# micknoise/Maximilian

Measured on AMD Instinct MI355X. Metric: Msamples/s (voice-bank render), higher is better.
Workload: dtype f64; 1 GPU; configs[1]: 65536-voice maxiOsc::sinebuf bank, block 512, out[n][v] stored, 8 rotated buffers; voices_per_gpu=65536, block=512, parallelism=units sharded x1, mixdown=off

## Files before the change

### maximilian_amd/csrc/mxg_pace.h

```cpp
#pragma once
#include "mxg_common.h"

namespace mxg {
namespace {

constexpr int kPaceWords = 8;
constexpr unsigned kPaceWindow = 32, kPaceLatesUp = 4, kPaceLatesDown = 1;
constexpr unsigned kPaceGaveUp = 0xffffffffu;

struct Pace {
    unsigned P, t0, k, late, cheap;
    __device__ __forceinline__ static unsigned now() { return (unsigned)__builtin_amdgcn_s_memrealtime(); }
    __device__ __forceinline__ void start(const unsigned *ctl, unsigned arg) {
        P = arg;
        if (ctl) {
            const unsigned p = __hip_atomic_load(ctl, __ATOMIC_RELAXED, __HIP_MEMORY_SCOPE_AGENT);
            if (p == kPaceGaveUp) P = 0;
            else if (p) P = p < 2 * arg ? p : 2 * arg;
        }
        k = late = cheap = 0;
        t0 = P ? now() : 0;
    }
    __device__ __forceinline__ void wait(bool is_cheap) {
        if (P) {
            const unsigned due = t0 + k * P;
            int d = (int)(now() - due);
            while (d < 0) {
                __builtin_amdgcn_s_sleep(1);
                d = (int)(now() - due);
            }
            late = (unsigned)d;
            k++;
            cheap += is_cheap ? 1u : 0u;
        }
    }
    __device__ __forceinline__ void finish(unsigned *ctl, unsigned arg, unsigned wg, unsigned nwg, bool tolerant = false) const {
        if (!ctl || !P || (wg & 15u)) return;
        const unsigned nrep = (nwg + 15u) / 16u;
        unsigned long long *acc = reinterpret_cast<unsigned long long *>(ctl + 4);
        const unsigned long long mine = ((unsigned long long)(late < 8 * P ? late : 8 * P) << 32) | ((unsigned long long)(k && cheap * 8 >= k * 7 ? 1u : 0u) << 16) | 1ull;
        const unsigned long long all = atomicAdd(acc, mine) + mine;
        if ((unsigned)(all & 0xffffu) != nrep) return;
        atomicExch(acc, 0ull);
        const unsigned worst = (unsigned)(all >> 32) / nrep, bound = (unsigned)((all >> 16) & 0xffffu);
        const unsigned c1 = atomicAdd(&ctl[1], 0u);
        unsigned p = P, w = c1 & 0xff, lates = (c1 >> 8) & 0xff, booted = (c1 >> 16) & 0xff, strikes = c1 >> 24;
        const unsigned up = tolerant ? 2 * kPaceLatesUp : kPaceLatesUp, down = tolerant ? 4 * kPaceLatesDown : kPaceLatesDown;
        if (bound * 8 >= nrep * 7) {
            const bool is_late = worst > p / 2;
            if (booted != 1) {
                strikes = is_late ? strikes + 1 : 0;
                if (booted == 0) {
                    if (is_late) {
                        booted = 2;
                        strikes = 0;
                    } else if (p > arg - arg / 4 + 1) {
                        p -= 2;
                    }
                } else if (strikes >= (tolerant ? 2u : 1u)) {
                    p++;
                    booted = 1;
                } else if (!is_late && p > arg - arg / 4) {
                    p--;
                }
            } else {
                lates += is_late ? 1 : 0;
                ++w;
                if (lates >= up) {
                    p++;
                    w = lates = 0;
                } else if (w >= kPaceWindow) {
                    if (lates <= down && p > arg - arg / 4) p--;
                    w = lates = 0;
                }
            }
        }
        if (p > arg + arg / 2) p = kPaceGaveUp;
        atomicExch(&ctl[0], p);
        atomicExch(&ctl[1], w | (lates << 8) | (booted << 16) | (strikes << 24));
        atomicExch(&ctl[7], worst);
    }
};

constexpr unsigned kTrialPhase = 32, kTrialCandidates = 3, kTrialAgain = 16384 + 5 * kTrialPhase;

struct PaceTrial {
    unsigned t_begin, n, period, tag;
    unsigned verdict;
    __device__ __forceinline__ static unsigned candidate(unsigned arg, unsigned i) { return arg * (31u - 2u * i) / 32u; }
    __device__ __forceinline__ void start(const unsigned *T, unsigned arg, unsigned block_len) {
        t_begin = Pace::now();
        n = 0;
        period = 0;
        verdict = 0;
        tag = block_len & 0xffffu;
        if (T) {
            unsigned d = __hip_atomic_load(T, __ATOMIC_RELAXED, __HIP_MEMORY_SCOPE_AGENT);
            const unsigned w1 = __hip_atomic_load(T + 1, __ATOMIC_RELAXED, __HIP_MEMORY_SCOPE_AGENT);
            n = w1 & 0xffffu;
            if ((w1 >> 16) != tag) {
                n = 0;
                d = 0;
            }
            verdict = d;
            if (d) {
                period = d >= 2 ? (d < 2 * arg ? d : 2 * arg) : 0;
            } else {
                const unsigned ph = n / kTrialPhase;
                period = (ph >= 2 && ph < 2 + kTrialCandidates) ? candidate(arg, ph - 2) : 0;
            }
        }
    }
    __device__ __forceinline__ void finish(unsigned *T, unsigned arg, unsigned wg, unsigned nwg) const {
        if (!T || (wg & 15u)) return;
        if (verdict && n + 1 < kTrialAgain) {
            if (wg == 0) __hip_atomic_fetch_add(&T[1], 1u, __ATOMIC_RELAXED, __HIP_MEMORY_SCOPE_AGENT);
            return;
        }
        const unsigned nrep = (nwg + 15u) / 16u;
        unsigned long long *acc = reinterpret_cast<unsigned long long *>(T + 2);
        const unsigned long long all = atomicAdd(acc, 1ull) + 1ull;
        if ((unsigned)(all & 0xffffu) != nrep) return;
        atomicExch(acc, 0ull);
        unsigned d = atomicAdd(&T[0], 0u), nn = n + 1;
        if ((atomicAdd(&T[1], 0u) >> 16) != tag) d = 0;
        if (!d) {
            if (nn % kTrialPhase == 0) {
                const unsigned t_now = Pace::now(), ph = n / kTrialPhase, wall = t_now - atomicAdd(&T[8], 0u);
                atomicExch(&T[8], t_now);
                if (ph == 1) {
                    atomicExch(&T[4], wall);
                    atomicExch(&T[5], 0xffffffffu);
                    atomicExch(&T[6], 0u);
                } else if (ph >= 2) {
                    unsigned best = atomicAdd(&T[5], 0u), best_p = atomicAdd(&T[6], 0u);
                    const bool done = ph + 1 == 2 + kTrialCandidates;
                    if (wall < best) {
                        best = wall;
                        best_p = candidate(arg, ph - 2);
                        atomicExch(&T[5], best);
                        atomicExch(&T[6], best_p);
                    }
                    if (done) d = ((unsigned long long)best * 100 < (unsigned long long)atomicAdd(&T[4], 0u) * 98) ? best_p : 1u;
                }
            }
        } else if (nn >= kTrialAgain) {
            d = 0;
            nn = 0;
        }
        atomicExch(&T[0], d);
        atomicExch(&T[1], nn | (tag << 16));
    }
};

}
}
```

### maximilian_amd/csrc/osc.hip

```cpp
#include <type_traits>

#include "mxg_common.h"
#include "maxi_tables.h"
#include "mxg_sincos.h"
#include "mxg_osc.h"
#include "mxg_lanefold.h"
#include "mxg_pace.h"

namespace mxg {

namespace {

__device__ const double MAXI_SINE_TAB_D[MAXI_SINE_TAB_LEN] = MAXI_SINE_TAB_INIT;
__device__ const double MAXI_TRANS_TAB_D[MAXI_TRANS_TAB_LEN] = MAXI_TRANS_TAB_INIT;

__device__ const double MXG_SINTAB_D[MXG_SINTAB_LEN] = {MXG_SINTAB_VALUES};

template <int WF>
constexpr bool uses_sine() {
    return WF == MXG_OSC_SINEBUF || WF == MXG_OSC_SINEBUF4;
}
static_assert((kSineOddOff & 1) == 1 && kSineOddOff >= MAXI_SINE_TAB_LEN, "parity copy of the sine table");
static_assert(tab_copy<MXG_OSC_SINEBUF, 1>() >= MAXI_SINE_TAB_LEN, "sinebuf's table copy");
static_assert(tab_copy<MXG_OSC_SAWN, 1>() >= MAXI_TRANS_TAB_LEN, "sawn's table copy");
static_assert(kSb4Copy >= MAXI_SINE_TAB_LEN && (kSb4Copy - 2) * 8 > 255 * 8, "sinebuf4's table copies: disjoint, and out of a ds_read2_b64's reach");
template <int WF, int FL = 0>
constexpr int tab_len() {
    return (WF == MXG_OSC_SINEBUF4 && MXG_SB4_PAIRS) ? kSineOddOff + MAXI_SINE_TAB_LEN + 1
           : WF == MXG_OSC_SINEBUF4                  ? 4 * kSb4Copy
           : uses_sine<WF>()                         ? tab_copy<WF, FL>() + MAXI_SINE_TAB_LEN
                           : (WF == MXG_OSC_SAWN ? tab_copy<WF, FL>() + MAXI_TRANS_TAB_LEN
                                                 : ((WF == MXG_OSC_SINEWAVE || WF == MXG_OSC_COSWAVE) ? MXG_SINTAB_WIDE_LEN : 1));
}
template <int WF, int FL = 0>
__device__ __forceinline__ void load_tab(double *s_tab) {
    if constexpr (uses_sine<WF>()) {
        for (int i = threadIdx.x; i < MAXI_SINE_TAB_LEN; i += blockDim.x) {
            s_tab[i] = MAXI_SINE_TAB_D[i];
            if constexpr (WF == MXG_OSC_SINEBUF4 && MXG_SB4_PAIRS) s_tab[kSineOddOff + i] = MAXI_SINE_TAB_D[i];
            if constexpr (tab_copy<WF, FL>() != 0) s_tab[tab_copy<WF, FL>() + i] = MAXI_SINE_TAB_D[i];
            if constexpr (WF == MXG_OSC_SINEBUF4 && !MXG_SB4_PAIRS) {
                s_tab[kSb4Copy + i] = MAXI_SINE_TAB_D[i];
                s_tab[2 * kSb4Copy + i] = MAXI_SINE_TAB_D[i];
                s_tab[3 * kSb4Copy + i] = MAXI_SINE_TAB_D[i];
            }
        }
    } else if constexpr (WF == MXG_OSC_SAWN) {
        for (int i = threadIdx.x; i < MAXI_TRANS_TAB_LEN; i += blockDim.x) {
            s_tab[i] = MAXI_TRANS_TAB_D[i];
            if constexpr (tab_copy<WF, FL>() != 0) s_tab[tab_copy<WF, FL>() + i] = MAXI_TRANS_TAB_D[i];
        }
    } else if constexpr (WF == MXG_OSC_SINEWAVE || WF == MXG_OSC_COSWAVE) {
        for (int i = threadIdx.x; i < MXG_SINTAB_WIDE_LEN; i += blockDim.x) s_tab[i] = MXG_SINTAB_D[i & (MXG_SINTAB_LEN - 1)];
    }
}

template <int WF, int FL, int ST>
__device__ __forceinline__ void paced_chunk(Pace &pc, double &ph, double &hd, const OscPre &q, const double *s_tab, double *&o, size_t P) {
    double r[8];
    osc_tick_chunk<WF, 8, FL>(ph, hd, q, s_tab, s_tab, r);
#pragma unroll
    for (int u = 0; u < 8; u++) asm volatile("" : "+v"(r[u]));
    pc.wait(true);
#pragma unroll
    for (int u = 0; u < 8; u++) {
        store1<ST>(o, r[u]);
        o += P;
    }
    __builtin_amdgcn_sched_barrier(0);
}

template <int WF, bool FPS, int VPL, int ST, bool PX>
__global__ void osc_kernel(size_t V, size_t N, const double *__restrict__ freq,
                           const double *__restrict__ p1, const double *__restrict__ p2,
                           double *__restrict__ phase_io, double *__restrict__ hold_io,
                           double *__restrict__ out, double sr, PartSync psync, int xcd, int p1ps, int passes, size_t v_begin,
                           size_t v_end, size_t P, unsigned *__restrict__ pace_ctl, unsigned pace_arg, unsigned *__restrict__ trial) {
#ifndef MXG_K1_LEAN_MASK
#define MXG_K1_LEAN_MASK ((1 << MXG_OSC_SINEWAVE) | (1 << MXG_OSC_COSWAVE) | (1 << MXG_OSC_SINEBUF4) | (1 << MXG_OSC_SAWN))
#endif
    constexpr bool kLean = ((MXG_K1_LEAN_MASK >> WF) & 1) != 0;
    constexpr int kFL = kLean ? kTickLean : 0;
    __shared__ __attribute__((aligned(16))) double s_tab[tab_len<WF, kFL>()];
    constexpr bool kPre = tab_len<WF, kFL>() > 1;
    double ph0[VPL] = {}, hd0[VPL] = {}, f0[VPL] = {};
    if constexpr (kPre) {
        const size_t w0 = v_begin + ((size_t)xcd_block(blockIdx.x, gridDim.x, xcd) * blockDim.x + threadIdx.x) * VPL;
        const size_t wc = (w0 + VPL <= v_end) ? w0 : (v_end >= v_begin + VPL ? v_end - VPL : v_begin);
#pragma unroll
        for (int j = 0; j < VPL; j++) {
            const size_t w = wc + j < v_end ? wc + j : v_end - 1;
            ph0[j] = phase_io[w];
            hd0[j] = hold_io[w];
            f0[j] = FPS ? 0.0 : freq[w];
        }
    }
    if constexpr (tab_len<WF, kFL>() > 1) {
        load_tab<WF, kFL>(s_tab);
        __syncthreads();
    }
    for (int pass = 0; pass < passes; pass++) {
    const size_t v0 = v_begin + (((size_t)pass * gridDim.x + xcd_block(blockIdx.x, gridDim.x, xcd)) * blockDim.x + threadIdx.x) * VPL;
    if (v0 >= v_end) return;

    double ph[VPL], hd[VPL];
    OscPre q[VPL];
#pragma unroll
    for (int j = 0; j < VPL; j++) {
        const bool pre = kPre && pass == 0 && v0 + VPL <= v_end;
        ph[j] = pre ? ph0[j] : phase_io[v0 + j];
        hd[j] = pre ? hd0[j] : hold_io[v0 + j];
        double a = p1 ? p1[v0 + j] : 0.0, b = p2 ? p2[v0 + j] : 0.0;
        if constexpr (!FPS) {
            q[j] = osc_pre<WF>(pre ? f0[j] : freq[v0 + j], sr, a, b);
        } else {
            q[j].p1 = a;
            q[j].p2 = b;
        }
    }
    int *const part_ctr = gridDim.y > 1 ? part_counter(psync) : nullptr;
    if (blockIdx.y + 1 != gridDim.y) part_signal(part_ctr);
    const size_t plen = (N + gridDim.y - 1) / gridDim.y;
    const size_t nA = blockIdx.y * plen < N ? blockIdx.y * plen : N;
    const size_t nB = nA + plen < N ? nA + plen : N;
    if constexpr (!FPS) {
#pragma unroll 4
        for (size_t n = 0; n < nA; n++) {
#pragma unroll
            for (int j = 0; j < VPL; j++) osc_skip<WF>(ph[j], hd[j], q[j], s_tab, s_tab);
        }
    }
    double *o = out + nA * P + v0;
    const double *fp = freq + v0;
    const double *pp = (FPS && p1ps) ? p1 + v0 : nullptr;
#ifndef MXG_OSC_UNROLL
#define MXG_OSC_UNROLL 4
#endif

    bool trust = false;
    if constexpr ((WF == MXG_OSC_SINEWAVE || WF == MXG_OSC_COSWAVE) && !FPS) {
        bool ok = true;
#pragma unroll
        for (int j = 0; j < VPL; j++)
            ok = ok && q[j].inc >= 0.0 && q[j].inc < 1.0 && ph[j] >= 0.0 && ph[j] < 2.0 && (__double2hiint(ph[j]) | __double2hiint(q[j].inc)) >= 0;
        trust = __all(ok);
        if (trust) {
#pragma unroll
            for (int j = 0; j < VPL; j++) q[j].sk = sintab_k();
        }
    }
    PaceTrial tr;
    tr.start(trial, pace_arg, (unsigned)N);
    Pace pc;
    pc.start(trial ? nullptr : pace_ctl, trial ? tr.period : pace_arg);
    auto run = [&](auto trust_tag) {
        constexpr bool kTrust = decltype(trust_tag)::value;
        size_t n = nA;
        if constexpr (PX && VPL == 1 && !FPS) {
            double *op = out + (nA + (threadIdx.x & 1)) * P + (v0 & ~(size_t)1);
            if constexpr (!kLean) {
                if (pc.P) {
                    double *o8 = out + nA * P + v0;
                    for (; n + 8 <= nB; n += 8) paced_chunk<WF, kFL, 1>(pc, ph[0], hd[0], q[0], s_tab, o8, P);
                    op += (n - nA) * P;
                }
#pragma unroll 2
                for (; n + 2 <= nB; n += 2) {
                    const double r0 = osc_tick<WF, kTrust, kFL>(ph[0], hd[0], q[0], s_tab, s_tab);
                    const double r1 = osc_tick<WF, kTrust, kFL>(ph[0], hd[0], q[0], s_tab, s_tab);
                    store_pair_rows<ST, false>(op, r0, r1);
                    op += 2 * P;
                }
            } else {
                const unsigned pairs = (unsigned)((nB - nA) >> 1);
                for (unsigned k = 0; k < pairs; k++) {
                    const double r0 = osc_tick<WF, kTrust, kFL>(ph[0], hd[0], q[0], s_tab, s_tab);
                    const double r1 = osc_tick<WF, kTrust, kFL>(ph[0], hd[0], q[0], s_tab, s_tab);
                    store_pair_rows<ST>(op, r0, r1);
                    op += 2 * P;
                }
                n = nA + 2 * (size_t)pairs;
            }
            o = out + n * P + v0;
        }
        if constexpr (VPL == 1 && !FPS && !PX && !kLean) {
            if (pc.P) {
                for (; n + 8 <= nB; n += 8) paced_chunk<WF, kFL, ST>(pc, ph[0], hd[0], q[0], s_tab, o, P);
            }
        }
#pragma unroll MXG_OSC_UNROLL
        for (; n < nB; n++) {
            double r[VPL];
#pragma unroll
            for (int j = 0; j < VPL; j++) {
                if constexpr (FPS) q[j] = osc_pre<WF>(fp[j], sr, pp ? pp[j] : q[j].p1, q[j].p2);
                r[j] = osc_tick<WF, kTrust, kFL>(ph[j], hd[j], q[j], s_tab, s_tab);
            }
            if constexpr (VPL == 2)
                store2<ST>(o, r[0], r[1]);
            else
                store1<ST>(o, r[0]);
            o += P;
            if constexpr (FPS) {
                fp += V;
                if (pp) pp += V;
            }
        }
    };
    if constexpr ((WF == MXG_OSC_SINEWAVE || WF == MXG_OSC_COSWAVE) && !FPS) {
        if (trust) run(std::true_type{}); else run(std::false_type{});
    } else {
        run(std::false_type{});
    }
    if (blockIdx.y + 1 == gridDim.y && part_wait(part_ctr, psync)) {
#pragma unroll
        for (int j = 0; j < VPL; j++) {
            phase_io[v0 + j] = ph[j];
            hold_io[v0 + j] = hd[j];
        }
    }
    if (threadIdx.x == 0) {
        pc.finish(trial ? nullptr : pace_ctl, pace_arg, blockIdx.x, gridDim.x, WF == MXG_OSC_SINEBUF);
        tr.finish(trial, pace_arg, blockIdx.x, gridDim.x);
    }
    }
}


template <int WF, int STORE, int WIN>
__global__ __launch_bounds__(256) void osc_mix_kernel(size_t V, size_t N, const double *__restrict__ freq,
                                                      const double *__restrict__ p1, const double *__restrict__ p2,
                                                      double *__restrict__ phase_io, double *__restrict__ hold_io,
                                                      double *__restrict__ out, const double *__restrict__ pan,
                                                      double *__restrict__ partial, double sr, PartSync psync, int passes) {
    constexpr int kTab = tab_len<WF, kTickLean>();
    constexpr int kTabPad = (kTab + 1) & ~1;
    __shared__ __attribute__((aligned(16))) double s_all[kTabPad + 4 * kTileWave + 4 * WIN * 2 + 256];
    double *s_tab = s_all;
    load_tab<WF, kTickLean>(s_tab);
    const int lane = threadIdx.x & 63, wave = threadIdx.x >> 6;
    double *tile = s_all + kTabPad + wave * kTileWave;
    double *s_part = s_all + kTabPad + 4 * kTileWave;
    double *my_part = s_part + wave * (WIN * 2);
    double *s_dump = s_part + 4 * WIN * 2;
    for (int pass = 0; pass < passes; pass++) {
    const size_t wg = (size_t)pass * gridDim.x + blockIdx.x;
    if (wg * blockDim.x >= V) break;
    if (pass) __syncthreads();
    const size_t vraw = wg * blockDim.x + threadIdx.x;
    const bool live = vraw < V;
    const size_t v = live ? vraw : (STORE == 2 ? V - 2 + (vraw & 1) : V - 1);
    double ph = phase_io[v], hd = hold_io[v];
    double x = pan[v];
    if (x > 1) x = 1;
    if (x < 0) x = 0;
    const int ts = lane & 15, tq = lane >> 4;
    double gl[16], gr[16];
    tile[lane] = live ? sqrt(1.0 - x) : 0.0;
    tile[64 + lane] = live ? sqrt(x) : 0.0;
    __syncthreads();
#pragma unroll
    for (int j = 0; j < 16; j++) {
        gl[j] = tile[16 * tq + j];
        gr[j] = tile[64 + 16 * tq + j];
    }
    OscPre q = osc_pre<WF>(freq[v], sr, p1 ? p1[v] : 0.0, p2 ? p2[v] : 0.0);
    asm volatile("" : "+v"(ph), "+v"(hd));
    asm volatile("" : "+v"(q.inc), "+v"(q.k), "+v"(q.p1), "+v"(q.p2));
#pragma unroll
    for (int j = 0; j < 16; j++) asm volatile("" : "+v"(gl[j]), "+v"(gr[j]));
    __syncthreads();
    int *const part_ctr = gridDim.y > 1 ? part_counter(psync) : nullptr;
    if (blockIdx.y + 1 != gridDim.y) part_signal(part_ctr);
    const size_t plen = ((N + gridDim.y - 1) / gridDim.y + kMixChunk - 1) / kMixChunk * kMixChunk;
    const size_t nA = blockIdx.y * plen < N ? blockIdx.y * plen : N;
    const size_t nB = nA + plen < N ? nA + plen : N;
#pragma unroll 4
    for (size_t n = 0; n < nA; n++) osc_skip<WF>(ph, hd, q, s_tab, s_tab);
    double *tw = tile + tq * kTileQuarter + ts;
    const double2v *tr = reinterpret_cast<const double2v *>(tile + tq * kTileQuarter + ts * kTileRow);
    double *o = out + nA * V + v;
    double *op = out + (nA + (threadIdx.x & 1)) * V + (v & ~(size_t)1);
    for (size_t n0 = nA; n0 < nB; n0 += WIN) {
        const int span = (int)((nB - n0) < (size_t)WIN ? (nB - n0) : (size_t)WIN);
        auto tile_load = [&](double2v (&xv)[8]) {
#pragma unroll
            for (int k = 0; k < 8; k++) xv[k] = tr[k];
        };
        auto tile_products = [&](const double2v (&xv)[8], double &sl, double &sr2) {
            double pl[8], pr[8];
#pragma unroll
            for (int k = 0; k < 8; k++) {
                pl[k] = xv[k].x * gl[2 * k] + xv[k].y * gl[2 * k + 1];
                pr[k] = xv[k].x * gr[2 * k] + xv[k].y * gr[2 * k + 1];
            }
            sl = ((pl[0] + pl[1]) + (pl[2] + pl[3])) + ((pl[4] + pl[5]) + (pl[6] + pl[7]));
            sr2 = ((pr[0] + pr[1]) + (pr[2] + pr[3])) + ((pr[4] + pr[5]) + (pr[6] + pr[7]));
        };
        auto tile_fold = [&](double sl, double sr2) {
            const double t = fold32(sl, sr2);
            return fold16(t, t);
        };
        auto tile_value = [&](const double2v (&xv)[8]) {
            double sl, sr2;
            tile_products(xv, sl, sr2);
            return tile_fold(sl, sr2);
        };
        auto tile_put = [&](double t, int c0, int cnt) {
            double *dst = ((lane & 16) == 0 && ts < cnt) ? my_part + (c0 + ts) * 2 + (lane >> 5) : s_dump + threadIdx.x;
            *dst = t;
        };
        auto tile_sum = [&](const double2v (&xv)[8], int c0, int cnt) { tile_put(tile_value(xv), c0, cnt); };
        int c_first = 0;
        if constexpr (osc_has_pipe<WF>() && STORE != 1) {
            const int full = span / kMixChunk;
            if (full > 0) {
                OscPipe<kMixChunk> P;
                osc_pipe_phase<WF, kMixChunk>(ph, q, P);
                __builtin_amdgcn_sched_barrier(0);
                osc_pipe_fetch<WF, kMixChunk>(P, s_tab);
                double t_prev = 0.0;
                auto body = [&](int c, auto last_tag) {
                    constexpr bool kLast = decltype(last_tag)::value;
                    double r[kMixChunk];
                    auto S = [&](int j) {
                        if constexpr (STORE == 2) {
                            store_pair_rows<2>(op, r[2 * j], r[2 * j + 1]);
                            op += 2 * V;
                        }
                    };
                    __builtin_amdgcn_sched_barrier(0);
                    osc_pipe_finish<WF, kMixChunk>(P, r, hd);
                    __builtin_amdgcn_sched_barrier(0);
                    S(0);
#pragma unroll
                    for (int i = 0; i < kMixChunk; i++) tw[i * kTileRow] = r[i];
                    tile_put(t_prev, (c - 1) * kMixChunk, c > 0 ? kMixChunk : 0);
                    __builtin_amdgcn_fence(__ATOMIC_RELEASE, "wavefront");
                    __builtin_amdgcn_wave_barrier();
                    __builtin_amdgcn_fence(__ATOMIC_ACQUIRE, "wavefront");
                    double2v xv[8];
                    tile_load(xv);
                    __builtin_amdgcn_fence(__ATOMIC_RELEASE, "wavefront");
                    __builtin_amdgcn_wave_barrier();
                    __builtin_amdgcn_sched_barrier(0);
                    S(1);
                    __builtin_amdgcn_sched_barrier(0);
                    if constexpr (!kLast) {
                        osc_pipe_phase_half<WF, kMixChunk, 0>(ph, q, P);
                        __builtin_amdgcn_sched_barrier(0);
                        S(2);
                        __builtin_amdgcn_sched_barrier(0);
                        osc_pipe_phase_half<WF, kMixChunk, 1>(ph, q, P);
                        __builtin_amdgcn_sched_barrier(0);
                        S(3);
                        __builtin_amdgcn_sched_barrier(0);
                        osc_pipe_fetch<WF, kMixChunk>(P, s_tab);
                        __builtin_amdgcn_sched_barrier(0);
                    } else {
                        S(2);
                        S(3);
                    }
                    S(4);
                    __builtin_amdgcn_sched_barrier(0);
                    double vl, vr;
                    tile_products(xv, vl, vr);
                    __builtin_amdgcn_sched_barrier(0);
                    S(5);
                    __builtin_amdgcn_sched_barrier(0);
                    t_prev = tile_fold(vl, vr);
                    __builtin_amdgcn_sched_barrier(0);
                    S(6);
                    S(7);
                };
                for (int c = 0; c + 1 < full; c++) body(c, std::false_type{});
                body(full - 1, std::true_type{});
                tile_put(t_prev, (full - 1) * kMixChunk, kMixChunk);
// ... 322 lines not shown
        case 2: return osc_kernel<WF, false, 1, 0, true>;
        case 3: return osc_kernel<WF, false, 1, 2, true>;
        case 4: return osc_kernel<WF, false, 1, 1, true>;
        default: return osc_kernel<WF, false, 1, 0, false>;
    }
}

osc_fn pick_wf(int wf, bool fps, int vpl, int store) {
    switch (wf) {
        case 0: return pick<0>(fps, vpl, store);
        case 1: return pick<1>(fps, vpl, store);
        case 2: return pick<2>(fps, vpl, store);
        case 3: return pick<3>(fps, vpl, store);
        case 4: return pick<4>(fps, vpl, store);
        case 5: return pick<5>(fps, vpl, store);
        case 6: return pick<6>(fps, vpl, store);
        case 7: return pick<7>(fps, vpl, store);
        case 8: return pick<8>(fps, vpl, store);
        case 9: return pick<9>(fps, vpl, store);
        case 10: return pick<10>(fps, vpl, store);
        case 11: return pick<11>(fps, vpl, store);
    }
    return nullptr;
}

}

}

namespace mxg {
namespace {
constexpr size_t kPacedFrom = 90112, kPacedFromSinebuf = 122880, kPacedTo = 327680;
struct OscLaunch {
    int waveform = 0;
    size_t V = 0, N = 0, P = 0;
    const double *freq = nullptr, *p1 = nullptr, *p2 = nullptr;
    int fps = 0;
    double *phase = nullptr, *hold = nullptr, *out = nullptr;
    hipStream_t st = nullptr;
    bool pairs_ok = false;
    size_t v_begin = 0, v_end = 0;
    int vpl = 1, store = 0, xcd = 0;
    int split = 0, passes = 0, block = 256;
    bool paced = false;
    bool trial = false;
};

void osc_single_rule(OscLaunch &L, size_t count) {
    const int wf = L.waveform;
    const bool heavy = wf == MXG_OSC_SINEWAVE || wf == MXG_OSC_COSWAVE || wf == MXG_OSC_SINEBUF4;
    const bool table = wf == MXG_OSC_SINEBUF || wf == MXG_OSC_SAWN;
    const size_t bytes = count * L.N * sizeof(double);
    L.vpl = 1;
    L.store = 0;
    L.xcd = 0;
    L.passes = 0;
    if (L.pairs_ok) {
        if (heavy) {
            if (bytes >= ((size_t)32 << 20)) L.store = 3;
            L.xcd = count >= 262144 ? 1 : 0;
        } else if (bytes >= ((size_t)192 << 20)) {
            if (wf == MXG_OSC_SINEBUF && count >= 67584 && count < 88064) {
                L.store = 1;
                L.passes = 2;
            } else if (count >= (wf == MXG_OSC_SAWN ? 98304u : table ? 81920u : 65536u)) {
                L.vpl = 2;
                L.store = 2;
                L.xcd = count >= 262144 ? 1 : 0;
            } else {
                L.store = 3;
            }
        }
    }
}

int osc_launch(const OscLaunch &L) {
    int vpl = L.vpl, store = L.store, block = L.block ? L.block : 256;
    const bool fps = L.fps != 0;
    const size_t count = L.v_end - L.v_begin;
    if (count == 0) return MXG_OK;
    const bool pairs_ok = L.pairs_ok && !(L.v_begin & 1) && !(count & 1);
    if (!pairs_ok) vpl = 1;
    if (vpl == 2 && store > 2) store = 0;
    if (vpl == 1 && store >= 2 && !pairs_ok) store = store == 4 ? 1 : 0;
    osc_fn fn = pick_wf(L.waveform, fps, vpl, store);
    const size_t lanes = (count + vpl - 1) / vpl;
    int split = L.split;
    if (split == 0) {
        split = 1;
        const size_t waves = (lanes + 63) / 64;
        const int wf = L.waveform;
        const bool heavy = wf == MXG_OSC_SINEWAVE || wf == MXG_OSC_COSWAVE || wf == MXG_OSC_SINEBUF4;
        const bool table = heavy || wf == MXG_OSC_SINEBUF || wf == MXG_OSC_SAWN;
        if (!fps && heavy) split = waves >= 2048 ? 1 : 2;
        if (!fps && table && waves < 1024) {
            int want = 1;
            while (want < 8 && (size_t)(2 * want) * waves <= 1024 && (size_t)(2 * want) * 64 <= L.N) want *= 2;
            if (want > split) split = want;
        }
    }
    if (fps) split = 1;
    while (split > 1 && (size_t)(split - 1) * ((L.N + split - 1) / split) >= L.N) split--;
    int passes = L.passes > 0 ? L.passes : 1;
    if (split > 1) passes = 1;
    size_t nblk = (lanes + block - 1) / block;
    if ((size_t)passes > nblk) passes = (int)nblk;
    nblk = (nblk + passes - 1) / passes;
    dim3 grid((unsigned)nblk, (unsigned)split), blk((unsigned)block);
    PartSync psync;
    if (split > 1)
        if (int s = part_sync_get(L.st, (size_t)grid.x * ((block + 63) / 64), split, &psync)) return s;
    unsigned *pace_ctl = nullptr;
    unsigned pace_arg = 0;
    {
        const int knob = tune_get("osc_pace");
        const bool lean = ((MXG_K1_LEAN_MASK >> L.waveform) & 1) != 0;
        if (split == 1 && passes == 1 && !fps && vpl == 1 && !lean) {
            if (knob >= 2) {
                pace_arg = (unsigned)knob;
            } else if (L.paced) {
                pace_arg = pace_start_period(count * 8 * 8);
                unsigned *base = pace_words(SCR_OSC_PACE, L.st, 16 * kPaceWords);
                if (base && pace_arg) pace_ctl = base + kPaceWords * (L.waveform & 15);
                else pace_arg = 0;
            }
        }
    }
    unsigned *trial = nullptr;
    if (L.trial && !pace_arg && split == 1 && passes == 1 && !fps && vpl == 1 && store == 3 && tune_get("osc_pace") == 0) {
        unsigned *base = pace_words(SCR_OSC_PACE, L.st, 16 * kPaceWords);
        if (base && pace_start_period(count * 8 * 8)) {
            trial = base + kPaceWords * 14;
            pace_arg = pace_start_period(count * 8 * 8);
        }
    }
    KernelTimer kt("osc_kernel", L.st);
    hipLaunchKernelGGL(fn, grid, blk, 0, L.st, L.V, L.N, L.freq, L.p1, L.p2, L.phase, L.hold, L.out, (double)settings().sampleRate, psync,
                       L.xcd, L.fps == 2 ? 1 : 0, passes, L.v_begin, L.v_end, L.P ? L.P : L.V, pace_ctl, pace_arg, trial);
    return check_hip(hipGetLastError(), "osc_kernel launch");
}
}
}

extern "C" int mxg_debug_osc_pace(void *stream, unsigned *host) {
    hipStream_t st = mxg::resolve_stream(stream);
    unsigned *base = nullptr;
    bool fresh = false;
    if (int s = mxg::scratch_get(mxg::SCR_OSC_PACE, st, 16 * mxg::kPaceWords * sizeof(unsigned), (void **)&base, &fresh)) return s;
    if (fresh) MXG_HIP(hipMemsetAsync(base, 0, 16 * mxg::kPaceWords * sizeof(unsigned), st));
    MXG_HIP(hipStreamSynchronize(st));
    return mxg::check_hip(hipMemcpy(host, base, 16 * mxg::kPaceWords * sizeof(unsigned), hipMemcpyDeviceToHost), "pace words");
}

extern "C" int mxg_osc_render(int waveform, size_t V, size_t N, const double *d_freq, int fps,
                              const double *d_p1, const double *d_p2, double *d_phase,
                              double *d_outhold, double *d_out, void *stream) {
    return mxg_osc_render_pitch(waveform, V, N, d_freq, fps, d_p1, d_p2, d_phase, d_outhold, d_out, V * sizeof(double), stream);
}

extern "C" int mxg_osc_render_pitch(int waveform, size_t V, size_t N, const double *d_freq, int fps,
                                    const double *d_p1, const double *d_p2, double *d_phase,
                                    double *d_outhold, double *d_out, size_t out_pitch_bytes, void *stream) {
    using namespace mxg;
    if (int s = ensure_init()) return s;
    MXG_REQUIRE(out_pitch_bytes % sizeof(double) == 0 && out_pitch_bytes >= V * sizeof(double),
                "out_pitch_bytes must be a multiple of 8 and at least V * 8");
    const size_t P = out_pitch_bytes / sizeof(double);
    MXG_REQUIRE(waveform >= 0 && waveform <= 11, "unknown waveform");
    MXG_REQUIRE(d_freq && d_phase && d_outhold && d_out, "null device pointer");
    MXG_REQUIRE(waveform != MXG_OSC_PULSE || d_p1, "pulse needs d_p1 (duty)");
    MXG_REQUIRE(waveform != MXG_OSC_PHASORBETWEEN || (d_p1 && d_p2),
                "phasorBetween needs d_p1/d_p2 (start/end phase)");
    MXG_REQUIRE(fps >= 0 && fps <= 2 && (fps != 2 || d_p1), "fps is 0, 1 (d_freq [N][V]) or 2 (d_freq and d_p1 [N][V])");
    MXG_REQUIRE(N <= 0xffffffffull, "a block holds at most 2^32 - 1 samples per voice");
    if (V == 0 || N == 0) return MXG_OK;
    const bool pairs_ok = !fps && !(V & 1) && !(P & 1) && !(((uintptr_t)d_out) & 15);
    hipStream_t st = resolve_stream(stream);
    OscLaunch L0;
    L0.waveform = waveform; L0.V = V; L0.P = P; L0.N = N; L0.freq = d_freq; L0.fps = fps; L0.p1 = d_p1; L0.p2 = d_p2; L0.phase = d_phase;
    L0.hold = d_outhold; L0.out = d_out; L0.st = st; L0.pairs_ok = pairs_ok;
    int vpl = tune_get("osc_vpl"), store = tune_get("osc_store") - 1, xcd = tune_get("osc_xcd") - 1;
    const bool automatic = vpl == 0 && store < 0;
    const bool heavy = waveform == MXG_OSC_SINEWAVE || waveform == MXG_OSC_COSWAVE || waveform == MXG_OSC_SINEBUF4;
    const bool lean_wf = ((MXG_K1_LEAN_MASK >> waveform) & 1) != 0 || (waveform == MXG_OSC_SINEBUF && V < kPacedFromSinebuf);
    if (automatic && !fps && !lean_wf && xcd < 0 && tune_get("osc_pace") == 0 && tune_get("osc_passes") == 0 && tune_get("osc_split") == 0 &&
        tune_get("osc_plan") == 0 && V >= kPacedFrom && V <= kPacedTo && pace_start_period(V * 8 * 8) &&
        pace_words(SCR_OSC_PACE, st, 16 * kPaceWords)) {
        OscLaunch A = L0;
        A.v_begin = 0; A.v_end = V; A.vpl = 1; A.store = 1; A.xcd = 0; A.split = 1; A.passes = 1; A.block = 256; A.paced = true;
        return osc_launch(A);
    }
    int plan = tune_get("osc_plan");
    if (plan == 0) plan = (P % 262144) ? 2 : (V == 262144 ? 3 : 1);
    if (automatic && pairs_ok && !heavy && xcd < 0 && tune_get("osc_passes") == 0 && tune_get("osc_split") == 0 && plan != 1 &&
        V * N * sizeof(double) >= ((size_t)352 << 20)) {
        const size_t kPass = 98304;
        size_t k = V / kPass;
        size_t rest = V - k * kPass;
        if (k > 0 && rest > 0 && rest < 40960 && rest + kPass <= 131072) {
            k--;
            rest += kPass;
        }
        if (k > 0) {
            OscLaunch A = L0;
            A.v_begin = 0; A.v_end = k * kPass; A.vpl = 2; A.store = 2; A.xcd = plan == 3 ? 1 : 0; A.split = 1; A.passes = (int)k; A.block = 256;
            if (int s2 = osc_launch(A)) return s2;
        }
        if (rest > 0) {
            OscLaunch B = L0;
            B.v_begin = k * kPass; B.v_end = V;
            osc_single_rule(B, rest);
            if (int s2 = osc_launch(B)) return s2;
        }
        return MXG_OK;
    }
    OscLaunch A = L0;
    A.v_begin = 0; A.v_end = V;
    if (automatic) {
        osc_single_rule(A, V);
        if (xcd >= 0) A.xcd = xcd;
        A.trial = waveform == MXG_OSC_SINEBUF && !fps && V >= 57344 && V < 73728;
    } else {
        if (vpl == 0) vpl = 1;
        if (store < 0) {
            const size_t out_bytes = V * N * sizeof(double);
            const int nt_knob = tune_get("osc_nt");
            store = (nt_knob == 1 || (nt_knob == 2 && out_bytes > ((size_t)300 << 20) && out_bytes <= ((size_t)1200 << 20))) ? 1 : 0;
        }
        A.vpl = vpl; A.store = store; A.xcd = xcd < 0 ? 0 : xcd;
    }
    A.block = tune_get("osc_block");
    A.split = tune_get("osc_split");
    if (const int kp = tune_get("osc_passes")) A.passes = kp;
    return osc_launch(A);
}

namespace mxg {
namespace {
int osc_mix_launch(int waveform, size_t V, size_t N, const double *d_freq, const double *d_p1, const double *d_p2,
                   double *d_phase, double *d_outhold, double *d_out, const double *d_pan, double *d_rows, hipStream_t st) {
    const int block = 256;
    const size_t nblocks = (V + block - 1) / block;
    int store = 0;
    if (d_out) {
        const bool pairs_ok = !(V & 1) && !(((uintptr_t)d_out) & 15) && V >= 2;
        const int knob = tune_get("osc_mix_store");
        store = (pairs_ok && (knob == 2 || (knob == 0 && V * N * sizeof(double) >= ((size_t)32 << 20)))) ? 2 : 1;
    }
    int split = tune_get("osc_mix_split");
    if (split == 0) {
        split = 1;
        const bool table = waveform == MXG_OSC_SINEWAVE || waveform == MXG_OSC_COSWAVE || waveform == MXG_OSC_SINEBUF4 ||
                           waveform == MXG_OSC_SINEBUF || waveform == MXG_OSC_SAWN;
        const size_t waves = nblocks * 4;
        if (table && waves < 1024)
            while (split < 8 && (size_t)(2 * split) * waves <= 1024 && (size_t)(2 * split) * 64 <= N) split *= 2;
    }
    while (split > 1 && (size_t)(split - 1) * (((N + split - 1) / split + kMixChunk - 1) / kMixChunk * kMixChunk) >= N) split--;
    PartSync psync;
    if (split > 1)
        if (int s2 = part_sync_get(st, nblocks * 4, split, &psync)) return s2;
    int win = tune_get("osc_mix_win");
    if (win == 0) win = nblocks * (size_t)split > 512 ? 128 : 256;
    osc_mix_fn fn = pick_mix_wf(waveform, store, win);
    int passes = tune_get("osc_mix_passes");
    if (passes == 0) passes = 1;
    if (split > 1) passes = 1;
    if ((size_t)passes > nblocks) passes = (int)nblocks;
    const size_t grid_x = (nblocks + passes - 1) / passes;
    const int pc = tune_get("osc_mix_pc");
    if (split == 1 && (pc == 2 || (pc == 0 && nblocks >= 128))) {
        KernelTimer kt("osc_mix_kernel", st);
        int pcwin = tune_get("osc_mix_pcwin");
        if (pcwin == 0) pcwin = 512;
        hipLaunchKernelGGL(pick_mixpc_wf(waveform, store, pcwin), dim3((unsigned)grid_x), dim3(512), 0, st, V, N, d_freq, d_p1, d_p2, d_phase,
                           d_outhold, d_out, d_pan, d_rows, (double)settings().sampleRate, passes);
        return check_hip(hipGetLastError(), "osc_mixpc_kernel launch");
    }
    KernelTimer kt("osc_mix_kernel", st);
    hipLaunchKernelGGL(fn, dim3((unsigned)grid_x, (unsigned)split), dim3(block), 0, st, V, N, d_freq, d_p1, d_p2, d_phase,
                       d_outhold, d_out, d_pan, d_rows, (double)settings().sampleRate, psync, passes);
    return check_hip(hipGetLastError(), "osc_mix_kernel launch");
}
}
}

extern "C" size_t mxg_osc_mix_groups(size_t V) { return (V + 255) / 256; }

extern "C" int mxg_mix_rows_sum(size_t groups, size_t count, const double *d_rows, double *d_mix, void *stream) {
    using namespace mxg;
    if (int s = ensure_init()) return s;
    MXG_REQUIRE(d_mix && (d_rows || groups == 0), "null device pointer");
    if (count == 0) return MXG_OK;
    hipStream_t st = resolve_stream(stream);
    KernelTimer kt("mix_partials_kernel", st);
    hipLaunchKernelGGL(mix_partials_kernel, dim3((unsigned)((count + 63) / 64)), dim3(64 * kPartWaves), 0, st, groups, count, d_rows,
                       d_mix);
    return check_hip(hipGetLastError(), "mix_partials_kernel launch");
}

extern "C" int mxg_osc_render_mix_rows(int waveform, size_t V, size_t N, const double *d_freq, const double *d_p1,
                                       const double *d_p2, double *d_phase, double *d_outhold, double *d_out,
                                       const double *d_pan, double *d_rows, void *stream) {
    using namespace mxg;
    if (int s = ensure_init()) return s;
    MXG_REQUIRE(waveform >= 0 && waveform <= 11, "unknown waveform");
// ... 108 lines not shown
```

Before: 822,400 Msamples/s.

## Issue sine table and pace-control loads together before LDS stores in oscillator kernel

```diff
diff --git a/maximilian_amd/csrc/mxg_pace.h b/maximilian_amd/csrc/mxg_pace.h
--- a/maximilian_amd/csrc/mxg_pace.h
+++ b/maximilian_amd/csrc/mxg_pace.h
@@ -11,15 +11,23 @@
 struct Pace {
     unsigned P, t0, k, late, cheap;
     __device__ __forceinline__ static unsigned now() { return (unsigned)__builtin_amdgcn_s_memrealtime(); }
+    __device__ __forceinline__ static unsigned period_of(bool has_ctl, unsigned p, unsigned arg) {
+        if (has_ctl) {
+            if (p == kPaceGaveUp) return 0;
+            if (p) return p < 2 * arg ? p : 2 * arg;
+        }
+        return arg;
+    }
     __device__ __forceinline__ void start(const unsigned *ctl, unsigned arg) {
-        P = arg;
-        if (ctl) {
-            const unsigned p = __hip_atomic_load(ctl, __ATOMIC_RELAXED, __HIP_MEMORY_SCOPE_AGENT);
-            if (p == kPaceGaveUp) P = 0;
-            else if (p) P = p < 2 * arg ? p : 2 * arg;
-        }
+        P = period_of(ctl != nullptr, ctl ? request(ctl) : 0u, arg);
         k = late = cheap = 0;
         t0 = P ? now() : 0;
+    }
+    __device__ __forceinline__ static unsigned request(const unsigned *ctl) { return __hip_atomic_load(ctl, __ATOMIC_RELAXED, __HIP_MEMORY_SCOPE_AGENT); }
+    __device__ __forceinline__ void consume(bool has_ctl, unsigned p, unsigned arg, unsigned t_now) {
+        P = period_of(has_ctl, p, arg);
+        k = late = cheap = 0;
+        t0 = P ? t_now : 0;
     }
     __device__ __forceinline__ void wait(bool is_cheap) {
         if (P) {
@@ -85,18 +93,19 @@
 constexpr unsigned kTrialPhase = 32, kTrialCandidates = 3, kTrialAgain = 16384 + 5 * kTrialPhase;
 
 struct PaceTrial {
-    unsigned t_begin, n, period, tag;
+    unsigned n, period, tag;
     unsigned verdict;
     __device__ __forceinline__ static unsigned candidate(unsigned arg, unsigned i) { return arg * (31u - 2u * i) / 32u; }
-    __device__ __forceinline__ void start(const unsigned *T, unsigned arg, unsigned block_len) {
-        t_begin = Pace::now();
+    __device__ __forceinline__ static void request(const unsigned *T, unsigned &d, unsigned &w1) {
+        d = __hip_atomic_load(T, __ATOMIC_RELAXED, __HIP_MEMORY_SCOPE_AGENT);
+        w1 = __hip_atomic_load(T + 1, __ATOMIC_RELAXED, __HIP_MEMORY_SCOPE_AGENT);
+    }
+    __device__ __forceinline__ void consume(bool has_T, unsigned d, unsigned w1, unsigned arg, unsigned block_len) {
         n = 0;
         period = 0;
         verdict = 0;
         tag = block_len & 0xffffu;
-        if (T) {
-            unsigned d = __hip_atomic_load(T, __ATOMIC_RELAXED, __HIP_MEMORY_SCOPE_AGENT);
-            const unsigned w1 = __hip_atomic_load(T + 1, __ATOMIC_RELAXED, __HIP_MEMORY_SCOPE_AGENT);
+        if (has_T) {
             n = w1 & 0xffffu;
             if ((w1 >> 16) != tag) {
                 n = 0;
diff --git a/maximilian_amd/csrc/osc.hip b/maximilian_amd/csrc/osc.hip
--- a/maximilian_amd/csrc/osc.hip
+++ b/maximilian_amd/csrc/osc.hip
@@ -32,28 +32,77 @@
                            : (WF == MXG_OSC_SAWN ? tab_copy<WF, FL>() + MAXI_TRANS_TAB_LEN
                                                  : ((WF == MXG_OSC_SINEWAVE || WF == MXG_OSC_COSWAVE) ? MXG_SINTAB_WIDE_LEN : 1));
 }
+template <int WF>
+constexpr int tab_src_len() {
+    return uses_sine<WF>() ? MAXI_SINE_TAB_LEN : WF == MXG_OSC_SAWN ? MAXI_TRANS_TAB_LEN : (WF == MXG_OSC_SINEWAVE || WF == MXG_OSC_COSWAVE) ? MXG_SINTAB_WIDE_LEN : 0;
+}
+template <int WF>
+constexpr int kTabRegs = (tab_src_len<WF>() + 255) / 256 > 0 ? (tab_src_len<WF>() + 255) / 256 : 1;
+template <int WF>
+__device__ __forceinline__ void tab_request(double (&r)[kTabRegs<WF>], int base) {
+    constexpr int L = tab_src_len<WF>();
+#pragma unroll
+    for (int j = 0; j < kTabRegs<WF>; j++) {
+        const int i = base + threadIdx.x + j * blockDim.x, ic = i < L ? i : L - 1;
+        if constexpr (uses_sine<WF>()) r[j] = MAXI_SINE_TAB_D[ic];
+        else if constexpr (WF == MXG_OSC_SAWN) r[j] = MAXI_TRANS_TAB_D[ic];
+        else r[j] = MXG_SINTAB_D[ic & (MXG_SINTAB_LEN - 1)];
+    }
+}
+template <int WF, int FL = 0>
+__device__ __forceinline__ void tab_put(double *s_tab, const double (&r)[kTabRegs<WF>], int base) {
+#pragma unroll
+    for (int j = 0; j < kTabRegs<WF>; j++) {
+        const int i = base + threadIdx.x + j * blockDim.x;
+        if (i >= tab_src_len<WF>()) continue;
+        s_tab[i] = r[j];
+        if constexpr (uses_sine<WF>()) {
+            if constexpr (WF == MXG_OSC_SINEBUF4 && MXG_SB4_PAIRS) s_tab[kSineOddOff + i] = r[j];
+            if constexpr (tab_copy<WF, FL>() != 0) s_tab[tab_copy<WF, FL>() + i] = r[j];
+            if constexpr (WF == MXG_OSC_SINEBUF4 && !MXG_SB4_PAIRS) {
+                s_tab[kSb4Copy + i] = r[j];
+                s_tab[2 * kSb4Copy + i] = r[j];
+                s_tab[3 * kSb4Copy + i] = r[j];
+            }
+        } else if constexpr (WF == MXG_OSC_SAWN) {
+            if constexpr (tab_copy<WF, FL>() != 0) s_tab[tab_copy<WF, FL>() + i] = r[j];
+        }
+    }
+}
+template <int WF, int FL = 0>
+__device__ __forceinline__ void tab_rest(double *s_tab, double (&r)[kTabRegs<WF>]) {
+    for (int base = kTabRegs<WF> * blockDim.x; base < tab_src_len<WF>(); base += kTabRegs<WF> * blockDim.x) {
+        tab_request<WF>(r, base);
+        constexpr int R = kTabRegs<WF>;
+        static_assert(R == 3 || R == 4 || R == 17, "the statement below names every register of the batch");
+        if constexpr (R == 3) asm volatile("" : "+v"(r[0]), "+v"(r[1]), "+v"(r[2]));
+        if constexpr (R == 4) asm volatile("" : "+v"(r[0]), "+v"(r[1]), "+v"(r[2]), "+v"(r[3]));
+        if constexpr (R == 17)
+            asm volatile("" : "+v"(r[0]), "+v"(r[1]), "+v"(r[2]), "+v"(r[3]), "+v"(r[4]), "+v"(r[5]), "+v"(r[6]), "+v"(r[7]), "+v"(r[8]), "+v"(r[9]),
+                              "+v"(r[10]), "+v"(r[11]), "+v"(r[12]), "+v"(r[13]), "+v"(r[14]), "+v"(r[15]), "+v"(r[16]));
+        tab_put<WF, FL>(s_tab, r, base);
+    }
+}
 template <int WF, int FL = 0>
 __device__ __forceinline__ void load_tab(double *s_tab) {
-    if constexpr (uses_sine<WF>()) {
-        for (int i = threadIdx.x; i < MAXI_SINE_TAB_LEN; i += blockDim.x) {
-            s_tab[i] = MAXI_SINE_TAB_D[i];
-            if constexpr (WF == MXG_OSC_SINEBUF4 && MXG_SB4_PAIRS) s_tab[kSineOddOff + i] = MAXI_SINE_TAB_D[i];
-            if constexpr (tab_copy<WF, FL>() != 0) s_tab[tab_copy<WF, FL>() + i] = MAXI_SINE_TAB_D[i];
-            if constexpr (WF == MXG_OSC_SINEBUF4 && !MXG_SB4_PAIRS) {
-                s_tab[kSb4Copy + i] = MAXI_SINE_TAB_D[i];
-                s_tab[2 * kSb4Copy + i] = MAXI_SINE_TAB_D[i];
-                s_tab[3 * kSb4Copy + i] = MAXI_SINE_TAB_D[i];
-            }
-        }
-    } else if constexpr (WF == MXG_OSC_SAWN) {
-        for (int i = threadIdx.x; i < MAXI_TRANS_TAB_LEN; i += blockDim.x) {
-            s_tab[i] = MAXI_TRANS_TAB_D[i];
-            if constexpr (tab_copy<WF, FL>() != 0) s_tab[tab_copy<WF, FL>() + i] = MAXI_TRANS_TAB_D[i];
-        }
-    } else if constexpr (WF == MXG_OSC_SINEWAVE || WF == MXG_OSC_COSWAVE) {
-        for (int i = threadIdx.x; i < MXG_SINTAB_WIDE_LEN; i += blockDim.x) s_tab[i] = MXG_SINTAB_D[i & (MXG_SINTAB_LEN - 1)];
-    }
-}
+    if constexpr (tab_src_len<WF>() > 0) {
+        double r[kTabRegs<WF>];
+        tab_request<WF>(r, 0);
+        tab_put<WF, FL>(s_tab, r, 0);
+        tab_rest<WF, FL>(s_tab, r);
+    }
+}
+
+#ifndef MXG_K1_STAMPS
+#define MXG_K1_STAMPS 0
+#endif
+constexpr int kK1StampWG = 1024, kK1StampN = 12;
+#if MXG_K1_STAMPS
+__device__ unsigned long long g_k1_stamps[2 * kK1StampWG * kK1StampN];
+#define K1_STAMP(i) (k1_stamp[i] = __builtin_amdgcn_s_memrealtime())
+#else
+#define K1_STAMP(i) ((void)0)
+#endif
 
 template <int WF, int FL, int ST>
 __device__ __forceinline__ void paced_chunk(Pace &pc, double &ph, double &hd, const OscPre &q, const double *s_tab, double *&o, size_t P) {
@@ -82,6 +131,12 @@
     constexpr bool kLean = ((MXG_K1_LEAN_MASK >> WF) & 1) != 0;
     constexpr int kFL = kLean ? kTickLean : 0;
     __shared__ __attribute__((aligned(16))) double s_tab[tab_len<WF, kFL>()];
+#if MXG_K1_STAMPS
+    unsigned long long k1_stamp[kK1StampN] = {};
+#endif
+    K1_STAMP(0);
+    const unsigned parts = gridDim.y;
+    asm volatile("" ::"s"(N), "s"(p1), "s"(p2), "s"(out), "s"(sr), "s"(psync.ctrs), "s"(psync.err), "s"(passes), "s"(P), "s"(pace_arg), "s"(parts), "s"(gridDim.x), "s"(blockDim.x));
     constexpr bool kPre = tab_len<WF, kFL>() > 1;
     double ph0[VPL] = {}, hd0[VPL] = {}, f0[VPL] = {};
     if constexpr (kPre) {
@@ -95,10 +150,20 @@
             f0[j] = FPS ? 0.0 : freq[w];
         }
     }
-    if constexpr (tab_len<WF, kFL>() > 1) {
-        load_tab<WF, kFL>(s_tab);
+    double tabr[kTabRegs<WF>];
+    if constexpr (kPre) tab_request<WF>(tabr, 0);
+    const unsigned *const pace_src = trial ? trial : pace_ctl;
+    const unsigned *const pace_ld = pace_src ? pace_src : reinterpret_cast<const unsigned *>(phase_io);
+    unsigned pw0, pw1;
+    PaceTrial::request(pace_ld, pw0, pw1);
+    const unsigned t_now = Pace::now();
+    K1_STAMP(2);
+    if constexpr (kPre) {
+        tab_put<WF, kFL>(s_tab, tabr, 0);
+        tab_rest<WF, kFL>(s_tab, tabr);
         __syncthreads();
     }
+    K1_STAMP(1);
     for (int pass = 0; pass < passes; pass++) {
     const size_t v0 = v_begin + (((size_t)pass * gridDim.x + xcd_block(blockIdx.x, gridDim.x, xcd)) * blockDim.x + threadIdx.x) * VPL;
     if (v0 >= v_end) return;
@@ -118,9 +183,9 @@
             q[j].p2 = b;
         }
     }
-    int *const part_ctr = gridDim.y > 1 ? part_counter(psync) : nullptr;
-    if (blockIdx.y + 1 != gridDim.y) part_signal(part_ctr);
-    const size_t plen = (N + gridDim.y - 1) / gridDim.y;
+    int *const part_ctr = parts > 1 ? part_counter(psync) : nullptr;
+    if (blockIdx.y + 1 != parts) part_signal(part_ctr);
+    const size_t plen = parts == 1 ? N : (N + parts - 1) / parts;
     const size_t nA = blockIdx.y * plen < N ? blockIdx.y * plen : N;
     const size_t nB = nA + plen < N ? nA + plen : N;
     if constexpr (!FPS) {
@@ -149,10 +214,13 @@
             for (int j = 0; j < VPL; j++) q[j].sk = sintab_k();
         }
     }
+    K1_STAMP(6);
     PaceTrial tr;
-    tr.start(trial, pace_arg, (unsigned)N);
+    asm volatile("" : "+v"(pw0), "+v"(pw1));
+    tr.consume(trial != nullptr, pw0, pw1, pace_arg, (unsigned)N);
     Pace pc;
-    pc.start(trial ? nullptr : pace_ctl, trial ? tr.period : pace_arg);
+    pc.consume(!trial && pace_ctl, pw0, trial ? tr.period : pace_arg, t_now);
+    K1_STAMP(7);
     auto run = [&](auto trust_tag) {
         constexpr bool kTrust = decltype(trust_tag)::value;
         size_t n = nA;
@@ -161,7 +229,12 @@
             if constexpr (!kLean) {
                 if (pc.P) {
                     double *o8 = out + nA * P + v0;
-                    for (; n + 8 <= nB; n += 8) paced_chunk<WF, kFL, 1>(pc, ph[0], hd[0], q[0], s_tab, o8, P);
+                    for (; n + 8 <= nB; n += 8) {
+                        paced_chunk<WF, kFL, 1>(pc, ph[0], hd[0], q[0], s_tab, o8, P);
+#if MXG_K1_STAMPS
+                        if (n == nA) K1_STAMP(3);
+#endif
+                    }
                     op += (n - nA) * P;
                 }
 #pragma unroll 2
@@ -170,6 +243,9 @@
                     const double r1 = osc_tick<WF, kTrust, kFL>(ph[0], hd[0], q[0], s_tab, s_tab);
                     store_pair_rows<ST, false>(op, r0, r1);
                     op += 2 * P;
+#if MXG_K1_STAMPS
+                    if (n == nA) K1_STAMP(3);
+#endif
                 }
             } else {
                 const unsigned pairs = (unsigned)((nB - nA) >> 1);
@@ -185,7 +261,12 @@
         }
         if constexpr (VPL == 1 && !FPS && !PX && !kLean) {
             if (pc.P) {
-                for (; n + 8 <= nB; n += 8) paced_chunk<WF, kFL, ST>(pc, ph[0], hd[0], q[0], s_tab, o, P);
+                for (; n + 8 <= nB; n += 8) {
+                    paced_chunk<WF, kFL, ST>(pc, ph[0], hd[0], q[0], s_tab, o, P);
+#if MXG_K1_STAMPS
+                    if (n == nA) K1_STAMP(3);
+#endif
+                }
             }
         }
 #pragma unroll MXG_OSC_UNROLL
@@ -212,7 +293,8 @@
     } else {
         run(std::false_type{});
     }
-    if (blockIdx.y + 1 == gridDim.y && part_wait(part_ctr, psync)) {
+    K1_STAMP(4);
+    if (blockIdx.y + 1 == parts && part_wait(part_ctr, psync)) {
 #pragma unroll
         for (int j = 0; j < VPL; j++) {
             phase_io[v0 + j] = ph[j];
@@ -223,6 +305,18 @@
         pc.finish(trial ? nullptr : pace_ctl, pace_arg, blockIdx.x, gridDim.x, WF == MXG_OSC_SINEBUF);
         tr.finish(trial, pace_arg, blockIdx.x, gridDim.x);
     }
+#if MXG_K1_STAMPS
+    K1_STAMP(5);
+    if (threadIdx.x == 0 && blockIdx.x < kK1StampWG && blockIdx.y == 0 && pass == 0) {
+        unsigned long long *dst = g_k1_stamps + ((size_t)(tr.n & 1u) * kK1StampWG + blockIdx.x) * kK1StampN;
+#pragma unroll
+        for (int i = 0; i < 6; i++) dst[i] = k1_stamp[i];
+        dst[6] = k1_stamp[6];
+        dst[7] = k1_stamp[7];
+        dst[8] = pc.P;
+        dst[9] = tr.n;
+    }
+#endif
     }
 }
 
@@ -851,6 +945,16 @@
     return mxg::check_hip(hipMemcpy(host, base, 16 * mxg::kPaceWords * sizeof(unsigned), hipMemcpyDeviceToHost), "pace words");
 }
 
+extern "C" int mxg_debug_k1_stamps(void *stream, unsigned long long *host) {
+#if MXG_K1_STAMPS
+    MXG_HIP(hipStreamSynchronize(mxg::resolve_stream(stream)));
+    return mxg::check_hip(hipMemcpyFromSymbol(host, HIP_SYMBOL(mxg::g_k1_stamps), sizeof(unsigned long long) * 2 * mxg::kK1StampWG * mxg::kK1StampN),
+                          "k1 stamps");
+#else
+    return mxg::fail(MXG_ERR_INVALID, "%s: this library was built without MXG_K1_STAMPS", __func__);
+#endif
+}
+
 extern "C" int mxg_osc_render(int waveform, size_t V, size_t N, const double *d_freq, int fps,
                               const double *d_p1, const double *d_p2, double *d_phase,
                               double *d_outhold, double *d_out, void *stream) {
```

Result: slower. 803,900 Msamples/s (-2.3%).
